# fuine/katome

Hardware: AMD Instinct MI355X
Metric: k-mers/s (higher is better)
Workload: dtype u64

## Files before the change

### katome_amd/csrc/lds_count.hip

```cpp
#include <algorithm>
#include <vector>

#include "common.h"
#include "lds_order.h"
#include "lds_plan.h"
#include "s2_regions.h"
#include "slot_bits.h"

namespace katome {

#ifdef KATOME_LC_PHASES
__device__ unsigned long long lc_phase_cycles[16];
#define LC_PHASE_BEGIN() unsigned long long lc_t0 = clock64()
#define LC_PHASE(i) do { if (threadIdx.x == 0) { const unsigned long long lc_t = clock64(); atomicAdd(&lc_phase_cycles[i], lc_t - lc_t0); lc_t0 = lc_t; } } while (0)
__device__ unsigned long long lo_phase_cycles[8];
#define LO_PHASE_BEGIN() unsigned long long lo_t0 = clock64()
#define LO_PHASE(i) do { if (threadIdx.x == 0) { const unsigned long long lo_t = clock64(); atomicAdd(&lo_phase_cycles[i], lo_t - lo_t0); lo_t0 = lo_t; } } while (0)
#else
#define LC_PHASE_BEGIN() do {} while (0)
#define LC_PHASE(i) do {} while (0)
#define LO_PHASE_BEGIN() do {} while (0)
#define LO_PHASE(i) do {} while (0)
#endif
template <int PER> KD u32 lc_step(u64 h) {
#ifdef KATOME_LC_LINEAR
    return 1u;
#else
    u32 step = (u32)((h >> 33) & 0x1FFu) * 2u + 1u;
    if ((PER & (PER - 1)) != 0 && step % (u32)PER == 0) step += 2;
    return step;
#endif
}

template <int NW, int STRIDE = NW>
__global__ __launch_bounds__(BLOCK) void hash_group_index_kernel(const u64* __restrict__ keys, u64 n, u32 gbits, u64* __restrict__ index) {
    for (u64 g = (u64)blockIdx.x * BLOCK + threadIdx.x; g <= (1ull << gbits); g += (u64)gridDim.x * BLOCK) {
        u64 lo = 0, hi = n;
        while (lo < hi) {
            const u64 mid = lo + ((hi - lo) >> 1);
            Key<NW> a;
#pragma unroll
            for (int q = 0; q < NW; ++q) a.w[q] = keys[mid * STRIDE + q];
            if ((hash_key(a) >> (64 - gbits)) < g) lo = mid + 1; else hi = mid;
        }
        index[g] = lo;
    }
}

template <bool RC, int PER, bool EVEN_K>
__global__ __launch_bounds__(LC_THREADS) void lds_count_kernel(const u64* keys, const u32* wts, const u64* __restrict__ index, u32 gbits,
                                                                u32 R, u32 k, u32 min_weight, u64* out_keys,
                                                                u32* out_w, u64 out_cap, unsigned long long* cursor,
                                                                unsigned long long* distinct, u32* err, u32 probe_limit,
                                                                unsigned long long* owner_cursor, u32 n_owners) {
    constexpr u32 LC_SLOTS = LcTable<PER>::SLOTS;
    extern __shared__ unsigned long long lc_mem[];
    unsigned long long* lkey = lc_mem;
    u32* lcnt = reinterpret_cast<u32*>(lc_mem + LC_SLOTS);
    __shared__ u32 wtot[LC_THREADS / 64];
    __shared__ unsigned long long base_sh;
    const u32 tid = threadIdx.x, lane = tid & 63, wave = tid >> 6;
    u32 my_distinct = 0;
    LC_PHASE_BEGIN();
    const u32 n_groups = 1u << gbits, sub_shift = 64 - gbits - 16;
    for (u32 g = blockIdx.x; g < n_groups; g += gridDim.x) {
        const u64 lo = index[g], hi = index[g + 1];
        if (lo == hi) continue;
        for (u32 r = 0; r < R; ++r) {
            for (u32 i = tid; i < LC_SLOTS; i += LC_THREADS) { lkey[i] = 0ull; lcnt[i] = 0u; }
            __syncthreads();
            LC_PHASE(0);
            constexpr u32 LU = KATOME_LC_LU;
            for (u64 i0 = lo + tid; i0 < hi; i0 += (u64)LC_THREADS * LU) {
                u64 kv[LU]; u32 wv[LU];
#pragma unroll
                for (u32 u = 0; u < LU; ++u) { const u64 i = i0 + (u64)u * LC_THREADS; kv[u] = 0; wv[u] = 0; if (i < hi) { kv[u] = keys[i]; wv[u] = wts[i]; } }
#pragma unroll
                for (u32 u = 0; u < LU; ++u) {
                    const u64 i = i0 + (u64)u * LC_THREADS;
                    if (i >= hi) continue;
                    Key<1> key; key.w[0] = kv[u];
                    const u64 h = hash_key(key);
                    if (R > 1 && (u32)((((h >> sub_shift) & 0xFFFFull) * R) >> 16) != r) continue;
                    const unsigned long long want = key.w[0] | OCC;
                    u32 s = (u32)(((h & 0x3FFFFFFFull) * LC_SLOTS) >> 30);
                    const u32 step = lc_step<PER>(h);
                    u32 probes = 0;
                    for (; probes < probe_limit; ++probes) {
                        const unsigned long long cur = atomicCAS(&lkey[s], 0ull, want);
                        if (cur == 0ull || cur == want) { atomicAdd(&lcnt[s], wv[u]); break; }
                        s += step; if (s >= LC_SLOTS) s -= LC_SLOTS;
                    }
                    if (probes == probe_limit) *err = 3;
                }
            }
            __syncthreads();
            LC_PHASE(1);

            Key<1> kk[PER]; u32 cc[PER], ne[PER]; u32 mine = 0;
#pragma unroll
            for (u32 j = 0; j < PER; ++j) {
                const u32 sidx = tid * PER + j;
                const unsigned long long v = lkey[sidx];
                ne[j] = 0; cc[j] = 0; kk[j].w[0] = 0;
                if (v & OCC) {
                    kk[j].w[0] = v & KEYBITS; cc[j] = lcnt[sidx];
                    ++my_distinct;
                    ne[j] = RC ? 2 : 1;
                    if (RC && EVEN_K && key_eq(revcomp(kk[j], k), kk[j])) ne[j] = 1;
                    if ((cc[j] << ((RC && ne[j] == 1) ? 1u : 0u)) < min_weight) ne[j] = 0;
                }
                mine += ne[j];
            }
            u32 incl = mine;
#pragma unroll
            for (int o = 1; o < 64; o <<= 1) { u32 v = __shfl_up(incl, o, 64); if (lane >= (u32)o) incl += v; }
            if (lane == 63) wtot[wave] = incl;
            __syncthreads();
            u32 woff = 0, total = 0;
#pragma unroll
            for (u32 w = 0; w < LC_THREADS / 64; ++w) { if (w < wave) woff += wtot[w]; total += wtot[w]; }
            if (tid == 0) base_sh = !total ? 0ull : owner_cursor ? atomicAdd(&owner_cursor[core_group_owner(g, n_owners)], (unsigned long long)total)
                                                               : atomicAdd(cursor, (unsigned long long)total);
            __syncthreads();
            LC_PHASE(2);
            {
                unsigned long long* skey = lc_mem;
                u32* sw = lcnt;
                const u32 p0 = woff + (incl - mine);
                for (u32 c0 = 0; c0 < total; c0 += LC_SLOTS) {
                    u32 p = p0 - c0;
#pragma unroll
                    for (u32 j = 0; j < PER; ++j) {
                        if (!ne[j]) continue;
                        const u32 w = cc[j] << ((RC && ne[j] == 1) ? 1u : 0u);
                        if (p < LC_SLOTS) { skey[p] = kk[j].w[0]; sw[p] = w; }
                        ++p;
                        if (ne[j] == 2) {
                            if (p < LC_SLOTS) { skey[p] = revcomp(kk[j], k).w[0]; sw[p] = w; }
                            ++p;
                        }
                    }
                    __syncthreads();
                    const u32 nc = total - c0 < LC_SLOTS ? total - c0 : LC_SLOTS;
                    const u64 o0 = base_sh + c0;
                    for (u32 i = tid; i < nc; i += LC_THREADS)
                        if (o0 + i < out_cap) { out_keys[o0 + i] = skey[i]; out_w[o0 + i] = sw[i]; }
                    __syncthreads();
                }
            }
            LC_PHASE(3);
        }
    }
    my_distinct = wave_sum(my_distinct);
    if (lane == 0 && my_distinct) atomicAdd(distinct, (unsigned long long)my_distinct);
}

constexpr u32 LP_STAGE = LP_SLOTS * 8 / 12;
template <bool RC>
__global__ __launch_bounds__(LC_THREADS) void lds_count_packed_kernel(const u64* keys, const u32* wts, const u64* __restrict__ index, u32 R, u32 k,
                                                                       u32 min_weight, u64* out_keys, u32* out_w, u64 out_cap, unsigned long long* cursor,
                                                                       unsigned long long* distinct, u32* err, u32 probe_limit) {
    constexpr unsigned long long REM = (1ull << 48) - 1;
    extern __shared__ unsigned long long lc_mem[];
    unsigned long long* slot = lc_mem;
    __shared__ u32 wtot[LC_THREADS / 64];
    __shared__ unsigned long long base_sh;
    const u32 tid = threadIdx.x, lane = tid & 63, wave = tid >> 6;
    u32 my_distinct = 0;
    LC_PHASE_BEGIN();
    for (u32 g = blockIdx.x; g < (1u << 16); g += gridDim.x) {
        const u64 lo = index[g], hi = index[g + 1];
        if (lo == hi) continue;
        for (u32 r = 0; r < R; ++r) {
            for (u32 i = tid; i < LP_SLOTS; i += LC_THREADS) slot[i] = 0ull;
// ... 379 lines not shown
    for (u32 g = blockIdx.x; g < n_groups; g += gridDim.x) {
        const u64 lo = index[g], hi = index[g + 1];
        if (lo == hi) continue;
        if (hi - lo > REP_MASK) { if (tid == 0) *err = 4; continue; }
        for (u32 r = 0; r < R; ++r) {
            for (u32 i = tid; i < LC_SLOTS; i += LC_THREADS) { lkey[i] = 0ull; lcnt[i] = 0u; }
            __syncthreads();
            LC_PHASE(4);
            constexpr u32 LU = KATOME_LC_LU;
            Key<NW> kv[LU]; u32 wv[LU];
            auto fetch = [&](u64 i0, Key<NW>* kk, u32* ww) {
#pragma unroll
                for (u32 u = 0; u < LU; ++u) {
                    const u64 i = i0 + (u64)u * LC_THREADS;
                    ww[u] = 0;
#pragma unroll
                    for (int q = 0; q < NW; ++q) kk[u].w[q] = 0;
                    if (i < hi) {
#pragma unroll
                        for (int q = 0; q < NW; ++q) kk[u].w[q] = keys[i * NW + q];
                        ww[u] = wts ? wts[i] : 1u;
                    }
                }
            };
            fetch(lo + tid, kv, wv);
            for (u64 i0 = lo + tid; i0 < hi; i0 += (u64)LC_THREADS * LU) {
              Key<NW> kn[LU]; u32 wn[LU];
              fetch(i0 + (u64)LC_THREADS * LU, kn, wn);
#pragma unroll
              for (u32 u = 0; u < LU; ++u) {
                const u64 i = i0 + (u64)u * LC_THREADS;
                if (i >= hi) continue;
                const Key<NW> key = kv[u];
                const u64 h = hash_key(key);
                if (R > 1 && (u32)((((h >> sub_shift) & 0xFFFFull) * R) >> 16) != r) continue;
                const unsigned long long want = OCC | (((h >> 5) & ((1ull << 43) - 1)) << 20) | (unsigned long long)(i - lo);
                const u32 w = wv[u];
                u32 s = (u32)(((h & 0x3FFFFFFFull) * LC_SLOTS) >> 30);
                const u32 step = lc_step<PER>(h);
                u32 probes = 0;
                for (; probes < probe_limit; ++probes) {
                    const unsigned long long cur = atomicCAS(&lkey[s], 0ull, want);
                    bool mine = cur == 0ull;
                    if (!mine && (cur >> 20) == (want >> 20)) {
                        const u64 j = lo + (cur & REP_MASK);
                        mine = true;
#ifndef KATOME_LC_EXPERIMENT_NO_COMPARE
#pragma unroll
                        for (int q = 0; q < NW; ++q) mine = mine && keys[j * NW + q] == key.w[q];
#endif
                    }
                    if (mine) { atomicAdd(&lcnt[s], w); break; }
                    s += step; if (s >= LC_SLOTS) s -= LC_SLOTS;
                }
                if (probes == probe_limit) *err = 3;
              }
#pragma unroll
              for (u32 u = 0; u < LU; ++u) { kv[u] = kn[u]; wv[u] = wn[u]; }
            }
            __syncthreads();
            LC_PHASE(5);
            constexpr bool LOOK = RC && EVEN_K;
            u32 rp[PER], cc[PER], ne[PER]; u32 mine = 0;
#pragma unroll
            for (u32 j = 0; j < (u32)PER; ++j) {
                const u32 sidx = tid * PER + j;
                const unsigned long long v = lkey[sidx];
                ne[j] = 0; cc[j] = 0; rp[j] = 0;
                if (v & OCC) {
                    rp[j] = (u32)(v & REP_MASK);
                    cc[j] = lcnt[sidx];
                    ++my_distinct;
                    ne[j] = RC ? 2 : 1;
                    if (LOOK) {
                        Key<NW> x;
#pragma unroll
                        for (int q = 0; q < NW; ++q) x.w[q] = keys[(lo + rp[j]) * NW + q];
                        if (key_eq(revcomp(x, k), x)) ne[j] = 1;
                    }
                    if ((cc[j] << ((RC && ne[j] == 1) ? 1u : 0u)) < min_weight) ne[j] = 0;
                }
                mine += ne[j];
            }
            u32 incl = mine;
#pragma unroll
            for (int o = 1; o < 64; o <<= 1) { u32 v = __shfl_up(incl, o, 64); if (lane >= (u32)o) incl += v; }
            if (lane == 63) wtot[wave] = incl;
            __syncthreads();
            u32 woff = 0, total = 0;
#pragma unroll
            for (u32 w = 0; w < LC_THREADS / 64; ++w) { if (w < wave) woff += wtot[w]; total += wtot[w]; }
            if (tid == 0) base_sh = total ? atomicAdd(cursor, (unsigned long long)total) : 0ull;
            __syncthreads();
            LC_PHASE(6);
            {
                constexpr u32 SC = LC_SLOTS * 12 / (8 * NW + 4);
                unsigned long long* skey = lc_mem;
                u32* sw = reinterpret_cast<u32*>(lc_mem + (size_t)SC * NW);
                const u32 p0 = woff + (incl - mine);
                for (u32 c0 = 0; c0 < total; c0 += SC) {
                    u32 p = p0 - c0;
#pragma unroll
                    for (u32 j = 0; j < (u32)PER; ++j) {
                        if (!ne[j]) continue;
                        const u32 w = cc[j] << ((RC && ne[j] == 1) ? 1u : 0u);
                        if (p < SC || (ne[j] == 2 && p + 1 < SC)) {
                            Key<NW> x;
#pragma unroll
                            for (int q = 0; q < NW; ++q) x.w[q] = keys[(lo + rp[j]) * NW + q];
                            if (p < SC) {
#pragma unroll
                                for (int q = 0; q < NW; ++q) skey[p * NW + q] = x.w[q];
                                sw[p] = w;
                            }
                            if (ne[j] == 2 && p + 1 < SC) {
                                const Key<NW> rk = revcomp(x, k);
#pragma unroll
                                for (int q = 0; q < NW; ++q) skey[(p + 1) * NW + q] = rk.w[q];
                                sw[p + 1] = w;
                            }
                        }
                        p += ne[j];
                    }
                    __syncthreads();
                    const u32 nc = total - c0 < SC ? total - c0 : SC;
                    const u64 o0 = base_sh + c0;
                    const u64 room = o0 < out_cap ? out_cap - o0 : 0;
                    const u32 nk = (u32)(room < nc ? room : nc);
                    for (u32 i = tid; i < nk * NW; i += LC_THREADS) out_keys[o0 * NW + i] = skey[i];
                    for (u32 i = tid; i < nk; i += LC_THREADS) out_w[o0 + i] = sw[i];
                    __syncthreads();
                }
            }
            LC_PHASE(7);
        }
    }
    my_distinct = wave_sum(my_distinct);
    if (lane == 0 && my_distinct) atomicAdd(distinct, (unsigned long long)my_distinct);
}

constexpr u64 LF_SALT = 0x9E3779B97F4A7C15ull;
template <bool RC, bool EVEN_K, int LF_PER>
__global__ __launch_bounds__(LC_THREADS) void lds_count_full_kernel(const u64* keys, const u32* wts, const u64* __restrict__ index, u32 groups_run, u32 k,
                                                                     u32 min_weight, u64* out_keys, u32* out_w, u64 out_cap, unsigned long long* cursor,
                                                                     unsigned long long* distinct, u32* err, u32 probe_limit) {
    constexpr u32 LF_SLOTS = LfTable<LF_PER>::SLOTS;
    extern __shared__ unsigned long long lc_mem[];
    ulonglong2* slot = reinterpret_cast<ulonglong2*>(lc_mem);
    u32* lcnt = reinterpret_cast<u32*>(lc_mem + 2 * (size_t)LF_SLOTS);
    __shared__ u32 wtot[LC_THREADS / 64];
    __shared__ unsigned long long base_sh;
    const u32 tid = threadIdx.x, lane = tid & 63, wave = tid >> 6;
    u32 my_distinct = 0;
    for (u32 g = blockIdx.x; g < groups_run; g += gridDim.x) {
        const u64 lo = index[g], hi = index[g + 1];
        if (lo == hi) continue;
        for (u32 i = tid; i < LF_SLOTS; i += LC_THREADS) { slot[i] = make_ulonglong2(0ull, 0ull); lcnt[i] = 0u; }
        __syncthreads();
        constexpr u32 LU = KATOME_LC_LU;
        u64 ka[LU], kb[LU]; u32 wv[LU];
        auto fetch = [&](u64 i0, u64* a, u64* b, u32* w) {
#pragma unroll
            for (u32 u = 0; u < LU; ++u) {
                const u64 i = i0 + (u64)u * LC_THREADS;
                a[u] = 0; b[u] = 0; w[u] = 0;
                if (i < hi) { const ulonglong2 v = *reinterpret_cast<const ulonglong2*>(keys + 2 * i); a[u] = v.x; b[u] = v.y; w[u] = wts ? wts[i] : 1u; }
            }
        };
        fetch(lo + tid, ka, kb, wv);
        for (u64 i0 = lo + tid; i0 < hi; i0 += (u64)LC_THREADS * LU) {
            u64 na[LU], nb[LU]; u32 nwv[LU];
            fetch(i0 + (u64)LC_THREADS * LU, na, nb, nwv);
#pragma unroll
            for (u32 u = 0; u < LU; ++u) {
                if (i0 + (u64)u * LC_THREADS >= hi) continue;
                Key<2> key; key.w[0] = ka[u]; key.w[1] = kb[u];
                const u64 h = hash_key(key);
                const unsigned long long A = ka[u] | OCC, B = kb[u] ^ LF_SALT;
                if (B == 0ull) { *err = 7; continue; }
                u32 s = (u32)(((h & 0x3FFFFFFFull) * LF_SLOTS) >> 30);
                const u32 step = lc_step<LF_PER>(h);
                u32 probes = 0;
                for (; probes < probe_limit; ++probes) {
                    const ulonglong2 v = slot[s];
                    unsigned long long a = v.x, b = v.y;
                    if (a == 0ull) { a = atomicCAS(&slot[s].x, 0ull, A); if (a == 0ull) a = A; }
                    if (a == A && b == 0ull) { b = atomicCAS(&slot[s].y, 0ull, B); if (b == 0ull) b = B; }
                    if (a == A && b == B) { atomicAdd(&lcnt[s], wv[u]); break; }
                    s += step; if (s >= LF_SLOTS) s -= LF_SLOTS;
                }
                if (probes == probe_limit) *err = 3;
            }
#pragma unroll
            for (u32 u = 0; u < LU; ++u) { ka[u] = na[u]; kb[u] = nb[u]; wv[u] = nwv[u]; }
        }
        __syncthreads();
        Key<2> kk[LF_PER]; u32 cc[LF_PER], ne[LF_PER]; u32 mine = 0;
#pragma unroll
        for (u32 j = 0; j < LF_PER; ++j) {
            const ulonglong2 v = slot[tid * LF_PER + j];
            ne[j] = 0; cc[j] = 0; kk[j].w[0] = 0; kk[j].w[1] = 0;
            if (v.x) {
                kk[j].w[0] = v.x & ~OCC; kk[j].w[1] = v.y ^ LF_SALT;
                cc[j] = lcnt[tid * LF_PER + j];
                ++my_distinct;
                ne[j] = RC ? 2 : 1;
                if (RC && EVEN_K && key_eq(revcomp(kk[j], k), kk[j])) ne[j] = 1;
                if ((cc[j] << ((RC && ne[j] == 1) ? 1u : 0u)) < min_weight) ne[j] = 0;
            }
            mine += ne[j];
        }
        u32 incl = mine;
#pragma unroll
        for (int o = 1; o < 64; o <<= 1) { u32 t = __shfl_up(incl, o, 64); if (lane >= (u32)o) incl += t; }
        if (lane == 63) wtot[wave] = incl;
        __syncthreads();
        u32 woff = 0, total = 0;
#pragma unroll
        for (u32 w = 0; w < LC_THREADS / 64; ++w) { if (w < wave) woff += wtot[w]; total += wtot[w]; }
        if (tid == 0) base_sh = total ? atomicAdd(cursor, (unsigned long long)total) : 0ull;
        __syncthreads();
        {
            unsigned long long* skey = lc_mem;
            u32* sw = lcnt;
            const u32 p0 = woff + (incl - mine);
            for (u32 c0 = 0; c0 < total; c0 += LF_SLOTS) {
                u32 p = p0 - c0;
#pragma unroll
                for (u32 j = 0; j < LF_PER; ++j) {
                    if (!ne[j]) continue;
                    const u32 w = cc[j] << ((RC && ne[j] == 1) ? 1u : 0u);
                    if (p < LF_SLOTS) { skey[2 * (size_t)p] = kk[j].w[0]; skey[2 * (size_t)p + 1] = kk[j].w[1]; sw[p] = w; }
                    ++p;
                    if (ne[j] == 2) {
                        if (p < LF_SLOTS) { const Key<2> rk = revcomp(kk[j], k); skey[2 * (size_t)p] = rk.w[0]; skey[2 * (size_t)p + 1] = rk.w[1]; sw[p] = w; }
                        ++p;
                    }
                }
                __syncthreads();
                const u32 nc = total - c0 < LF_SLOTS ? total - c0 : LF_SLOTS;
                const u64 o0 = base_sh + c0;
                const u64 room = o0 < out_cap ? out_cap - o0 : 0;
                const u32 nk = (u32)(room < nc ? room : nc);
                for (u32 i = tid; i < nk * 2; i += LC_THREADS) out_keys[o0 * 2 + i] = skey[i];
                for (u32 i = tid; i < nk; i += LC_THREADS) out_w[o0 + i] = sw[i];
                __syncthreads();
            }
        }
    }
    my_distinct = wave_sum(my_distinct);
    if (lane == 0 && my_distinct) atomicAdd(distinct, (unsigned long long)my_distinct);
}

constexpr u64 LF_SALT2 = 0xD1B54A32D192ED03ull;
template <int PER>
__global__ __launch_bounds__(LC_THREADS) void lds_count_full3_kernel(const u64* keys, const u32* wts, const u64* __restrict__ index, u32 groups_run,
                                                                      u64* out_keys, u32* out_w, u64 out_cap, unsigned long long* cursor,
                                                                      unsigned long long* distinct, u32* err, u32 probe_limit) {
    constexpr u32 SLOTS = Lf3Table<PER>::SLOTS;
    extern __shared__ unsigned long long lc_mem[];
    unsigned long long* sa = lc_mem;
    unsigned long long* sb = lc_mem + SLOTS;
    unsigned long long* sc = lc_mem + 2 * (size_t)SLOTS;
    u32* lcnt = reinterpret_cast<u32*>(lc_mem + 3 * (size_t)SLOTS);
    __shared__ u32 wtot[LC_THREADS / 64];
    __shared__ unsigned long long base_sh;
    const u32 tid = threadIdx.x, lane = tid & 63, wave = tid >> 6;
    u32 my_distinct = 0;
    for (u32 g = blockIdx.x; g < groups_run; g += gridDim.x) {
        const u64 lo = index[g], hi = index[g + 1];
        if (lo == hi) continue;
        for (u32 i = tid; i < SLOTS; i += LC_THREADS) { sa[i] = 0ull; sb[i] = 0ull; sc[i] = 0ull; lcnt[i] = 0u; }
        __syncthreads();
        constexpr u32 LU = 2;
        for (u64 i0 = lo + tid; i0 < hi; i0 += (u64)LC_THREADS * LU) {
            u64 ka[LU], kb[LU], kc[LU]; u32 wv[LU];
#pragma unroll
            for (u32 u = 0; u < LU; ++u) {
                const u64 i = i0 + (u64)u * LC_THREADS;
                ka[u] = 0; kb[u] = 0; kc[u] = 0; wv[u] = 0;
                if (i < hi) { ka[u] = keys[3 * i]; kb[u] = keys[3 * i + 1]; kc[u] = keys[3 * i + 2]; wv[u] = wts ? wts[i] : 1u; }
            }
#pragma unroll
            for (u32 u = 0; u < LU; ++u) {
                if (i0 + (u64)u * LC_THREADS >= hi) continue;
                Key<3> key; key.w[0] = ka[u]; key.w[1] = kb[u]; key.w[2] = kc[u];
                const u64 h = hash_key(key);
                const unsigned long long A = ka[u] | OCC, B = kb[u] ^ LF_SALT, C = kc[u] ^ LF_SALT2;
                if (B == 0ull || C == 0ull) { *err = 7; continue; }
                u32 s = (u32)(((h & 0x3FFFFFFFull) * SLOTS) >> 30);
                const u32 step = lc_step<PER>(h);
                u32 probes = 0;
                for (; probes < probe_limit; ++probes) {
                    unsigned long long a = sa[s], b = sb[s], c = sc[s];
                    if (a == 0ull) { a = atomicCAS(&sa[s], 0ull, A); if (a == 0ull) a = A; }
                    if (a == A && b == 0ull) { b = atomicCAS(&sb[s], 0ull, B); if (b == 0ull) b = B; }
                    if (a == A && b == B && c == 0ull) { c = atomicCAS(&sc[s], 0ull, C); if (c == 0ull) c = C; }
                    if (a == A && b == B && c == C) { atomicAdd(&lcnt[s], wv[u]); break; }
                    s += step; if (s >= SLOTS) s -= SLOTS;
                }
                if (probes == probe_limit) *err = 3;
            }
        }
        __syncthreads();
        Key<3> kk[PER]; u32 cc[PER]; u32 keep = 0;
#pragma unroll
        for (u32 j = 0; j < (u32)PER; ++j) {
            const u32 x = tid * PER + j;
            const unsigned long long a = sa[x];
            kk[j].w[0] = 0; kk[j].w[1] = 0; kk[j].w[2] = 0; cc[j] = 0;
            if (a) { kk[j].w[0] = a & ~OCC; kk[j].w[1] = sb[x] ^ LF_SALT; kk[j].w[2] = sc[x] ^ LF_SALT2; cc[j] = lcnt[x]; keep |= 1u << j; ++my_distinct; }
        }
        const u32 mine = (u32)__popc(keep);
        u32 incl = mine;
#pragma unroll
        for (int o = 1; o < 64; o <<= 1) { u32 t = __shfl_up(incl, o, 64); if (lane >= (u32)o) incl += t; }
        if (lane == 63) wtot[wave] = incl;
        __syncthreads();
        u32 woff = 0, total = 0;
#pragma unroll
        for (u32 w = 0; w < LC_THREADS / 64; ++w) { if (w < wave) woff += wtot[w]; total += wtot[w]; }
        if (tid == 0) base_sh = total ? atomicAdd(cursor, (unsigned long long)total) : 0ull;
        __syncthreads();
        {
            unsigned long long* skey = lc_mem;
            u32* sw = lcnt;
            u32 p = woff + (incl - mine);
#pragma unroll
            for (u32 j = 0; j < (u32)PER; ++j) {
                if (!((keep >> j) & 1u)) continue;
                skey[3 * (size_t)p] = kk[j].w[0]; skey[3 * (size_t)p + 1] = kk[j].w[1]; skey[3 * (size_t)p + 2] = kk[j].w[2]; sw[p] = cc[j];
                ++p;
            }
            __syncthreads();
            const u64 o0 = base_sh;
            const u64 room = o0 < out_cap ? out_cap - o0 : 0;
            const u32 nk = (u32)(room < total ? room : total);
            for (u32 i = tid; i < nk * 3; i += LC_THREADS) out_keys[o0 * 3 + i] = skey[i];
            for (u32 i = tid; i < nk; i += LC_THREADS) out_w[o0 + i] = sw[i];
            __syncthreads();
        }
    }
    my_distinct = wave_sum(my_distinct);
    if (lane == 0 && my_distinct) atomicAdd(distinct, (unsigned long long)my_distinct);
}

template <bool RC, int NWK, bool LIST = false, bool DELTA = false>
__global__ __launch_bounds__(LC_THREADS) void lds_count_seen_kernel(const u64* recs, const u32* wts, const u64* __restrict__ index, u32 gbits, u32 R, u32 k,
                                                                     u64 seq_per_read, u64* out_keys, u64* out_pairs, u64 out_cap,
                                                                     unsigned long long* cursor, unsigned long long* distinct, u32* err, u32 probe_limit) {
    constexpr u32 SLOTS = LC_THREADS * LCS_PER;
    constexpr int STRIDE = NWK + 1;
    constexpr unsigned long long REP_MASK = (1ull << 20) - 1;
    extern __shared__ unsigned long long lcs_mem[];
    unsigned long long* lkey = lcs_mem;
    unsigned long long* lA = lcs_mem + SLOTS;
    unsigned long long* lB = lcs_mem + 2 * SLOTS;
    u32* lcnt = reinterpret_cast<u32*>(lcs_mem + 3 * SLOTS);
    __shared__ u32 wtot[LC_THREADS / 64];
    __shared__ unsigned long long base_sh;
    const u32 tid = threadIdx.x, lane = tid & 63, wave = tid >> 6;
    u32 my_distinct = 0;
    const u32 n_groups = 1u << gbits, sub_shift = 64 - gbits - 16;
    for (u32 g = blockIdx.x; g < n_groups; g += gridDim.x) {
        const u64 lo = index[g], hi = index[g + 1];
        if (lo == hi) continue;
        if (NWK > 1 && hi - lo > REP_MASK) { if (tid == 0) *err = 4; continue; }
        for (u32 r = 0; r < R; ++r) {
            for (u32 i = tid; i < SLOTS; i += LC_THREADS) { lkey[i] = 0ull; lA[i] = SEEN_NONE; lB[i] = SEEN_NONE; lcnt[i] = 0u; }
            __syncthreads();
            constexpr u32 LU = 4;
            for (u64 i0 = lo + tid; i0 < hi; i0 += (u64)LC_THREADS * LU) {
              Key<NWK> kv[LU]; unsigned long long tv[LU]; u32 wv[LU];
#pragma unroll
              for (u32 u = 0; u < LU; ++u) {
                  const u64 i = i0 + (u64)u * LC_THREADS;
                  tv[u] = 0; wv[u] = 0;
#pragma unroll
                  for (int q = 0; q < NWK; ++q) kv[u].w[q] = 0;
                  if (i < hi) {
#pragma unroll
                      for (int q = 0; q < NWK; ++q) kv[u].w[q] = recs[i * STRIDE + q];
                      tv[u] = recs[i * STRIDE + NWK]; wv[u] = wts ? wts[i] : 1u;
                  }
              }
#pragma unroll
              for (u32 u = 0; u < LU; ++u) {
                const u64 i = i0 + (u64)u * LC_THREADS;
                if (i >= hi) continue;
                const Key<NWK> key = kv[u];
                const u64 h = hash_key(key);
                if (R > 1 && (u32)((((h >> sub_shift) & 0xFFFFull) * R) >> 16) != r) continue;
                const unsigned long long tag = tv[u];
                const unsigned long long want = NWK == 1 ? (OCC | key.w[0]) : (OCC | (((h >> 5) & ((1ull << 43) - 1)) << 20) | (unsigned long long)(i - lo));
                const u32 w = wv[u];
                u32 s = (u32)(((h & 0x3FFFFFFFull) * SLOTS) >> 30);
                const u32 step = lc_step<LCS_PER>(h);
                u32 probes = 0;
                for (; probes < probe_limit; ++probes) {
                    const unsigned long long cur = atomicCAS(&lkey[s], 0ull, want);
                    bool mine = cur == 0ull || (NWK == 1 && cur == want);
// ... 454 lines not shown
    template <int PER> using Table = Lf3Table<PER>;
    static constexpr int SMALL = 3, LARGE = 5, SLOT_BYTES = 28;
    static constexpr const char* WHAT = "whole three-word keys";
    template <int PER, class... A> static int launch(const LcLevel& c, size_t lds, LcResult& r, u32 groups, A... tail) {
        return lc_launch(c.aux, lds_count_full3_kernel<PER>, lds, c.n, r, c.ko, c.wo, c.index, groups, tail...);
    }
};
template <class T> static int count_whole_keys(const LcLevel& c, LcResult& r, bool* done) {
    typedef typename T::template Table<T::SMALL> Small; typedef typename T::template Table<T::LARGE> Large;
    if (c.split || c.gbits != 16) return KATOME_OK;
    auto count = [&](u32 groups, u64 cap, bool small) {
        auto go = [&](auto per) {
            typedef typename T::template Table<decltype(per)::value> Tab;
            return T::template launch<decltype(per)::value>(c, (size_t)Tab::SLOTS * T::SLOT_BYTES, r, groups, c.out_keys, c.out_w, cap, c.aux.cursor(), c.aux.distinct(),
                                                            c.aux.err(), std::min<u32>(lc_probe_limit(), Tab::SLOTS));
        };
        return small ? go(IntC<T::SMALL>{}) : go(IntC<T::LARGE>{});
    };
    const u32 all = 1u << c.gbits, sample = 256u;
    bool take = lc_full_mode() == 1, small = lc_full_per() == 4;
    if (lc_full_mode() < 0 && c.avg > 0 && c.avg <= 8ull * Large::FILL) {
        KCHECK(count(sample, 0, false));
        const u64 per_group = r.n_distinct / sample;
        take = r.code == 0 && per_group <= Large::FILL;
        if (!lc_full_per()) small = lf_small_table(per_group, Small::SLOTS);
    }
    if (!take) return KATOME_OK;
    KCHECK(count(all, c.out_cap, small));
    lc_trace("[lds count] %s in the slots (%d per thread): code %u\n", T::WHAT, small ? T::SMALL : T::LARGE, (unsigned)r.code);
    if (r.code == 3 && small) {
        KCHECK(count(all, c.out_cap, false));
        lc_trace("[lds count] %s in the slots (%d per thread): code %u\n", T::WHAT, T::LARGE, (unsigned)r.code);
    }
    *done = r.code == 0;
    return KATOME_OK;
}

static int count_packed(const LcLevel& c, u32 R_try, LcResult& r, bool* done) {
    static const int packed_mode = env_int("KATOME_LC_PACKED", 1);
    if (c.nw != 1 || c.split || !c.wo || c.gbits != 16 || !(R_try > 1 || packed_mode == 2) || (c.rc && (c.k & 1) == 0)) return KATOME_OK;
    const u32 R_p = lp_rounds(c.avg);
    if (!(packed_mode == 2 || (packed_mode && R_p < R_try))) return KATOME_OK;
    KCHECK(with_bool(c.rc, [&](auto rcv) {
        return lc_launch(c.aux, lds_count_packed_kernel<decltype(rcv)::value>, (size_t)LP_SLOTS * 8, c.n, r, c.ko, c.wo, c.index, R_p, c.k, c.min_weight, c.out_keys,
                         c.out_w, c.out_cap, c.aux.cursor(), c.aux.distinct(), c.aux.err(), std::min<u32>(lc_probe_limit(), LP_SLOTS));
    }));
    lc_trace("[lds count] 8-byte slots, %u visit(s) per record: code %u\n", R_p, (unsigned)r.code);
    *done = r.code == 0;
    if (r.code) lc_trace("[lds count] 8-byte slots: %s; counting with the 12-byte slots\n", r.code == 5 ? "a count beyond 16 bits" : "a table filled");
    return KATOME_OK;
}

int records_to_edges_sorted(DevBuf& keys, DevBuf& weights, uint64_t n, uint32_t k, bool rc, uint32_t min_weight, DevBuf& edge_key,
                            DevBuf& edge_weight, uint64_t* n_edges, uint64_t* n_distinct, hipStream_t stream, OwnerSplit* split,
                            uint32_t* first_counts, HalfSort* half, RecordSource* src) {
    *n_edges = 0; *n_distinct = 0;
    auto records = [&]() { return src && src->pending ? table_materialise_records(*src) : (int)KATOME_OK; };
    if (half) {
        half->taken = false;
        if (split) KCHECK(records());
        const int orc = split ? KATOME_E_UNSUPPORTED : ordered_count(keys, weights, n, k, rc, min_weight, *half, n_edges, n_distinct, stream, first_counts, src);
        if (orc != KATOME_E_UNSUPPORTED) return orc;
        if (rc) KCHECK(table_orient_records(keys.as<u64>(), n, k, false, stream));
        first_counts = nullptr;
    }
    const uint32_t nw = (uint32_t)key_words_for_k(k);
    if (nw > 3 || (nw == 3 && (rc || min_weight))) { KCHECK(records()); return KATOME_E_UNSUPPORTED; }
    if (split && (nw != 1 || rc || min_weight || split->n_parts == 0 || split->n_parts > (uint32_t)KATOME_MAX_RANKS)) {
        set_error("records by owner: one-word k-mers, one record per k-mer"); return KATOME_E_ARG;
    }
    if (!lc_level_fits(n, LcTable<13>::FILL)) { KCHECK(records()); return KATOME_E_UNSUPPORTED; }
    if (split) KCHECK(records());
    LcAux aux(stream);
    LcLevel c{aux};
    c.n = n; c.k = k; c.nw = nw; c.rc = rc; c.min_weight = min_weight; c.split = split;
    const bool unit = weights.p == nullptr && !(src && src->pending);
    if (unit && (nw < 2 || split)) { set_error("records without weights: keys of two or three words"); return KATOME_E_ARG; }
    {
        DevBuf kb(stream), wb(stream);
        KCHECK(kb.alloc((n + 1) * 8 * nw));
        if (!unit) KCHECK(wb.alloc((n + 1) * 4));
        if (split) KCHECK(dev_hash_order_core(keys.as<u64>(), weights.as<u32>(), n, split->core_shift, split->core_bases, kb.as<u64>(), keys.as<u64>(), wb.as<u32>(),
                                              weights.as<u32>(), &c.ko, &c.wo, &c.gbits, stream));
        else KCHECK(dev_hash_order(keys.as<u64>(), weights.as<u32>(), n, nw, kb.as<u64>(), keys.as<u64>(), wb.as<u32>(), weights.as<u32>(), &c.ko, &c.wo, &c.gbits, stream, first_counts, src));
    }
    c.avg = n >> c.gbits;
    const u32 fill = c.avg <= LcTable<8>::FILL ? LcTable<8>::FILL : LcTable<13>::FILL;
    const u32 R = lc_rounds(c.avg, fill);
    if (R > LC_MAX_ROUNDS) return KATOME_E_UNSUPPORTED;
    DevBuf index(stream);
    KCHECK(index.alloc(((1ull << c.gbits) + 1) * 8));
    KCHECK(aux.buf.alloc(64));
    c.index = index.as<u64>();
    {
        KernelScope ks(K_GROUP_INDEX, stream, n);
        const dim3 igrid(grid_for((1ull << c.gbits) + 1, BLOCK));
        if (split)   hipLaunchKernelGGL(core_group_index_kernel, igrid, dim3(BLOCK), 0, stream, c.ko, n, c.gbits, split->core_shift, split->core_bases, index.as<u64>());
        else if (nw == 1) hipLaunchKernelGGL(hash_group_index_kernel<1>, igrid, dim3(BLOCK), 0, stream, c.ko, n, c.gbits, index.as<u64>());
        else if (nw == 3) hipLaunchKernelGGL(hash_group_index_kernel<3>, igrid, dim3(BLOCK), 0, stream, c.ko, n, c.gbits, index.as<u64>());
        else         hipLaunchKernelGGL(hash_group_index_kernel<2>, igrid, dim3(BLOCK), 0, stream, c.ko, n, c.gbits, index.as<u64>());
    }
    c.out_cap = (rc ? 2 : 1) * n + 1;
    KCHECK(edge_key.alloc(c.out_cap * 8 * nw, stream));
    KCHECK(edge_weight.alloc(c.out_cap * 4, stream));
    c.out_keys = edge_key.as<u64>(); c.out_w = edge_weight.as<u32>();
    if (split) {
        KCHECK(aux.owners.alloc((2 * KATOME_MAX_RANKS + 2) * 8));
        aux.index = c.index; aux.gbits = c.gbits; aux.n_owners = split->n_parts;
    }
    LcResult r;
    bool done = false;
    if (nw == 2) KCHECK(count_whole_keys<WholeKeys2>(c, r, &done));
    if (nw == 3) KCHECK(count_whole_keys<WholeKeys3>(c, r, &done));
    const u32 R_try = lc_rounds_try(c.avg, lc_optimism(), fill);
    if (!done) KCHECK(count_packed(c, R_try, r, &done));
    if (!done) {
        KCHECK(count_optimistic("packed key", R_try, R, ~0u, r, [&](u32 rounds, u32 probe_limit) { return count_sub_rounds(c, rounds, probe_limit, r); }));
        if (r.code == 4) return KATOME_E_UNSUPPORTED;
        if (r.code) { set_error("counting in LDS: a sub-round did not fit its table (code %u)", (unsigned)r.code); return KATOME_E_DEVICE; }
    }
    *n_edges = r.n_out; *n_distinct = r.n_distinct;
    if (split) {
        uint64_t hb[2 * KATOME_MAX_RANKS + 2];
        KCHECK_HIP(hipMemcpyAsync(hb, aux.owners.p, sizeof hb, hipMemcpyDeviceToHost, stream));
        KCHECK_HIP(hipStreamSynchronize(stream));
        uint64_t total = 0;
        for (uint32_t p = 0; p < split->n_parts; ++p) {
            split->base[p] = hb[KATOME_MAX_RANKS + 1 + p];
            split->count[p] = hb[p] - split->base[p];
            total += split->count[p];
        }
        *n_edges = total;
    }
    return KATOME_OK;
}

}

#ifdef KATOME_LC_PHASES
extern "C" int katome_debug_lc_phases(uint64_t* out16) {
    unsigned long long h[16];
    if (hipMemcpyFromSymbol(h, HIP_SYMBOL(katome::lc_phase_cycles), sizeof h) != hipSuccess) return -1;
    for (int i = 0; i < 16; ++i) out16[i] = h[i];
    memset(h, 0, sizeof h);
    return hipMemcpyToSymbol(HIP_SYMBOL(katome::lc_phase_cycles), h, sizeof h) == hipSuccess ? 0 : -1;
}
extern "C" int katome_debug_lo_phases(uint64_t* out8) {
    unsigned long long h[8];
    if (hipMemcpyFromSymbol(h, HIP_SYMBOL(katome::lo_phase_cycles), sizeof h) != hipSuccess) return -1;
    for (int i = 0; i < 8; ++i) out8[i] = h[i];
    memset(h, 0, sizeof h);
    return hipMemcpyToSymbol(HIP_SYMBOL(katome::lo_phase_cycles), h, sizeof h) == hipSuccess ? 0 : -1;
}
#endif
```

Measured before the change: 177.9 billion.

## Prefetch next group's keys across group seam in LDS count kernel

Restructures the group loop in the full LDS counting kernel so the next group's index bounds are read early and its first key batch is fetched before the current group's compaction and output phase. Empty groups are skipped ahead of time, and one __syncthreads before the cursor atomicAdd is dropped, relying on the later barrier inside the output loop. The aim is to hide global load latency at group boundaries and cut a barrier, at the cost of extra live registers. Prefetch is disabled for the RC, LF_PER=7 variant. The change also adds optional phase-timing instrumentation behind a debug macro.

```diff
diff --git a/katome_amd/csrc/lds_count.hip b/katome_amd/csrc/lds_count.hip
--- a/katome_amd/csrc/lds_count.hip
+++ b/katome_amd/csrc/lds_count.hip
@@ -16,11 +16,18 @@
 __device__ unsigned long long lo_phase_cycles[8];
 #define LO_PHASE_BEGIN() unsigned long long lo_t0 = clock64()
 #define LO_PHASE(i) do { if (threadIdx.x == 0) { const unsigned long long lo_t = clock64(); atomicAdd(&lo_phase_cycles[i], lo_t - lo_t0); lo_t0 = lo_t; } } while (0)
+__device__ unsigned long long seam_phase_cycles[16];
+#define SEAM_PHASE_BEGIN() unsigned long long sm_t0 = clock64()
+#define SEAM_PHASE(i) do { if (threadIdx.x == 0) { const unsigned long long sm_t = clock64(); atomicAdd(&seam_phase_cycles[i], sm_t - sm_t0); sm_t0 = sm_t; } } while (0)
+#define SEAM_ARRIVED(x) do { if ((x) == 0xFFFFFFFEu) atomicAdd(&seam_phase_cycles[15], 1ull); } while (0)
 #else
 #define LC_PHASE_BEGIN() do {} while (0)
 #define LC_PHASE(i) do {} while (0)
 #define LO_PHASE_BEGIN() do {} while (0)
 #define LO_PHASE(i) do {} while (0)
+#define SEAM_PHASE_BEGIN() do {} while (0)
+#define SEAM_PHASE(i) do {} while (0)
+#define SEAM_ARRIVED(x) do {} while (0)
 #endif
 template <int PER> KD u32 lc_step(u64 h) {
 #ifdef KATOME_LC_LINEAR
@@ -706,25 +713,40 @@
     __shared__ unsigned long long base_sh;
     const u32 tid = threadIdx.x, lane = tid & 63, wave = tid >> 6;
     u32 my_distinct = 0;
-    for (u32 g = blockIdx.x; g < groups_run; g += gridDim.x) {
-        const u64 lo = index[g], hi = index[g + 1];
-        if (lo == hi) continue;
+    constexpr u32 LU = KATOME_LC_LU;
+    u64 ka[LU], kb[LU]; u32 wv[LU];
+    auto fetch = [&](u64 i0, u64 end, u64* a, u64* b, u32* w) {
+#pragma unroll
+        for (u32 u = 0; u < LU; ++u) {
+            const u64 i = i0 + (u64)u * LC_THREADS;
+            a[u] = 0; b[u] = 0; w[u] = 0;
+            if (i < end) { const ulonglong2 v = *reinterpret_cast<const ulonglong2*>(keys + 2 * i); a[u] = v.x; b[u] = v.y; w[u] = wts ? wts[i] : 1u; }
+        }
+    };
+    auto skip_empty = [&](u32& g, u64& lo, u64& hi) {
+        while (g < groups_run && lo == hi) {
+            g += gridDim.x;
+            if (g < groups_run) { lo = index[g]; hi = index[g + 1]; }
+        }
+    };
+    u32 g = blockIdx.x; u64 lo = 0, hi = 0;
+    if (g < groups_run) { lo = index[g]; hi = index[g + 1]; }
+    skip_empty(g, lo, hi);
+    constexpr bool TURN_AHEAD = !(RC && LF_PER == 7);
+    if (TURN_AHEAD && g < groups_run) fetch(lo + tid, hi, ka, kb, wv);
+    SEAM_PHASE_BEGIN();
+    while (g < groups_run) {
+        u32 ng = g + gridDim.x; u64 nlo = 0, nhi = 0;
+        if (ng < groups_run) { nlo = index[ng]; nhi = index[ng + 1]; }
+        if (!TURN_AHEAD) fetch(lo + tid, hi, ka, kb, wv);
         for (u32 i = tid; i < LF_SLOTS; i += LC_THREADS) { slot[i] = make_ulonglong2(0ull, 0ull); lcnt[i] = 0u; }
         __syncthreads();
-        constexpr u32 LU = KATOME_LC_LU;
-        u64 ka[LU], kb[LU]; u32 wv[LU];
-        auto fetch = [&](u64 i0, u64* a, u64* b, u32* w) {
-#pragma unroll
-            for (u32 u = 0; u < LU; ++u) {
-                const u64 i = i0 + (u64)u * LC_THREADS;
-                a[u] = 0; b[u] = 0; w[u] = 0;
-                if (i < hi) { const ulonglong2 v = *reinterpret_cast<const ulonglong2*>(keys + 2 * i); a[u] = v.x; b[u] = v.y; w[u] = wts ? wts[i] : 1u; }
-            }
-        };
-        fetch(lo + tid, ka, kb, wv);
+        SEAM_PHASE(1);
+        SEAM_ARRIVED(wv[LU - 1]);
+        SEAM_PHASE(2);
         for (u64 i0 = lo + tid; i0 < hi; i0 += (u64)LC_THREADS * LU) {
             u64 na[LU], nb[LU]; u32 nwv[LU];
-            fetch(i0 + (u64)LC_THREADS * LU, na, nb, nwv);
+            fetch(i0 + (u64)LC_THREADS * LU, hi, na, nb, nwv);
 #pragma unroll
             for (u32 u = 0; u < LU; ++u) {
                 if (i0 + (u64)u * LC_THREADS >= hi) continue;
@@ -749,6 +771,10 @@
             for (u32 u = 0; u < LU; ++u) { ka[u] = na[u]; kb[u] = nb[u]; wv[u] = nwv[u]; }
         }
         __syncthreads();
+        SEAM_PHASE(3);
+        skip_empty(ng, nlo, nhi);
+        SEAM_PHASE(0);
+        if (TURN_AHEAD && ng < groups_run) fetch(nlo + tid, nhi, ka, kb, wv);
         Key<2> kk[LF_PER]; u32 cc[LF_PER], ne[LF_PER]; u32 mine = 0;
 #pragma unroll
         for (u32 j = 0; j < LF_PER; ++j) {
@@ -772,8 +798,8 @@
         u32 woff = 0, total = 0;
 #pragma unroll
         for (u32 w = 0; w < LC_THREADS / 64; ++w) { if (w < wave) woff += wtot[w]; total += wtot[w]; }
-        if (tid == 0) base_sh = total ? atomicAdd(cursor, (unsigned long long)total) : 0ull;
-        __syncthreads();
+        SEAM_PHASE(4);
+        if (tid == 0 && total) base_sh = atomicAdd(cursor, (unsigned long long)total);
         {
             unsigned long long* skey = lc_mem;
             u32* sw = lcnt;
@@ -791,7 +817,9 @@
                         ++p;
                     }
                 }
+                SEAM_PHASE(6);
                 __syncthreads();
+                SEAM_PHASE(5);
                 const u32 nc = total - c0 < LF_SLOTS ? total - c0 : LF_SLOTS;
                 const u64 o0 = base_sh + c0;
                 const u64 room = o0 < out_cap ? out_cap - o0 : 0;
@@ -801,6 +829,8 @@
                 __syncthreads();
             }
         }
+        SEAM_PHASE(6);
+        g = ng; lo = nlo; hi = nhi;
     }
     my_distinct = wave_sum(my_distinct);
     if (lane == 0 && my_distinct) atomicAdd(distinct, (unsigned long long)my_distinct);
@@ -1561,4 +1591,11 @@
     memset(h, 0, sizeof h);
     return hipMemcpyToSymbol(HIP_SYMBOL(katome::lo_phase_cycles), h, sizeof h) == hipSuccess ? 0 : -1;
 }
+extern "C" int katome_debug_seam_phases(uint64_t* out16) {
+    unsigned long long h[16];
+    if (hipMemcpyFromSymbol(h, HIP_SYMBOL(katome::seam_phase_cycles), sizeof h) != hipSuccess) return -1;
+    for (int i = 0; i < 16; ++i) out16[i] = h[i];
+    memset(h, 0, sizeof h);
+    return hipMemcpyToSymbol(HIP_SYMBOL(katome::seam_phase_cycles), h, sizeof h) == hipSuccess ? 0 : -1;
+}
 #endif
```

Result: no change. 178.9 billion, median of 6 (+0.6%).
